# evoldoers/historian

Measured on AMD Instinct MI355X. Metric: forward-DP cells/s, higher is better.
Workload: dtype f64; 1 GPU; batch of independent 2x2000-residue protein leaf-profile pairs, WAG, t=0.2/0.3, full (unbanded) Forward DP; scaled-probability recursion with the reference's truncation: every pairwise sum of the reference's left-nested log_sum_exp drops a term that is at most e^-10 of the other, as the reference's table does (src/logsumexp.h:45); no table, log-probabilities at the store; lpEnd within 1e-9 rel. of; pairs_per_gpu=512, pairs_total=512, parallelism=pairs farmed across 1 rank(s); RCCL broadcast of model constants only

## Files before the change

### historian_amd/csrc/hx_linear.hip

```cpp
#include <hip/hip_runtime.h>
#include <cstdlib>
#include "hx_device.h"
#include "hx_lse.h"
#include "hx_common.h"
#include "hx_policy.h"
#include "hx_kernels.h"

namespace hx {

namespace {

#define HXL_PUBLISH_LAG 16
#define HX_YL_MAX_CLS_LINEAR 64
#define HXL_EMIN (-(1 << 28))
#define HXL_RENORM_MASK 6

struct L5 { double imm, imd, idm, imi, iiw; int e; };

#define HXL_EXP_M10 4.5399929762484854e-05
__device__ __forceinline__ double trunc_sum(double a, double b) {
  const double hi = fmax_plain(a, b), lo = fmin_plain(a, b);
  const int keep = lo > hi * HXL_EXP_M10 ? __double2hiint(lo) : 0;
  return hi + __hiloint2double(keep, __double2loint(lo));
}
template <bool TRUNC> __device__ __forceinline__ double lin_acc(double m, double p, double acc) {
  if (TRUNC) return trunc_sum(acc, m * p);
  return __builtin_fma(m, p, acc);
}

__device__ __forceinline__ L5 l5_zero() { return L5{0., 0., 0., 0., 0., HXL_EMIN}; }

__device__ __forceinline__ int dpp_shr1_keep0(int old, int v) {
  return __builtin_amdgcn_update_dpp(old, v, 0x138, 0xf, 0xf, false);
}
__device__ __forceinline__ double dpp_shr1_keep0(double old, double v) {
  const int lo = __builtin_amdgcn_update_dpp(__double2loint(old), __double2loint(v), 0x138, 0xf, 0xf, false);
  const int hi = __builtin_amdgcn_update_dpp(__double2hiint(old), __double2hiint(v), 0x138, 0xf, 0xf, false);
  return __hiloint2double(hi, lo);
}
__device__ __forceinline__ L5 dpp_shr1_old(const L5& o, const L5& c) {
  return L5{dpp_shr1_keep0(o.imm, c.imm), dpp_shr1_keep0(o.imd, c.imd), dpp_shr1_keep0(o.idm, c.idm),
            dpp_shr1_keep0(o.imi, c.imi), dpp_shr1_keep0(o.iiw, c.iiw), dpp_shr1_keep0(o.e, c.e)};
}

#define HXL_LOG_ENTRIES 1536
typedef double log_entry __attribute__((ext_vector_type(2)));
__device__ __forceinline__ log_entry log_issue(double m, const HX_LDS double* ltab) {
  const double f = __builtin_amdgcn_frexp_mant(m);
  unsigned idx;
  asm("v_bfe_u32 %0, %1, 11, 11" : "=v"(idx) : "v"(__double2hiint(f)));
  return *(const HX_LDS log_entry*)((const HX_LDS char*)ltab + (idx << 4));
}
__device__ __forceinline__ double log_finish(double m, int e, log_entry ce) {
  const double f = __builtin_amdgcn_frexp_mant(m);
  const int k = __builtin_amdgcn_frexp_exp(m);
  const double r = __builtin_fma(f, ce.x, -1.0);
  double p = __builtin_fma(r, 1.0 / 3.0, -0.5);
  p = __builtin_fma(p, r, 1.0);
  const double lf = __builtin_fma(p, r, ce.y);
  return __builtin_fma((double)(e + k), 0.693147180559945309417, lf);
}
__device__ __forceinline__ double log_scaled(double m, int e, const HX_LDS double* ltab) { return log_finish(m, e, log_issue(m, ltab)); }

__device__ __forceinline__ L5 from_logs(double a, double b, double c, double d, double g) {
  const double mx = vmax(vmax(vmax(a, b), vmax(c, d)), g);
  if (!(mx > HX_NEG_INF)) return l5_zero();
  const double n = __builtin_rint(mx * 1.44269504088896340736);
  const double hi = n * 0.693147180369123816490, lo = n * 1.90821492927058770002e-10;
  L5 r;
  r.imm = exp((a - hi) - lo);
  r.imd = exp((b - hi) - lo);
  r.idm = exp((c - hi) - lo);
  r.imi = exp((d - hi) - lo);
  r.iiw = exp((g - hi) - lo);
  r.e = (int)n;
  return r;
}

struct LdsPlan { int elds, ycol, yclass, flags, zero;
                 int a0, b0, a1, stride, total; };

#define HXL_RING 64
#define HXL_STAGE 128

#define HXL_PATIENCE (1 << 22)
template <int W, bool BANDED, int PPW, int DIR, bool MULTI = false, bool TRUNC = false>
__global__ void __launch_bounds__(W * PPW * 64, 4)
k_fill_leaf_linear(const DevJob* __restrict__ jobs, const double* __restrict__ exact_tab, const double* __restrict__ log_tab,
                      const LdsPlan plan, const int n_jobs, const int groups = 1, int* const counters = nullptr) {
  static_assert(!MULTI || (!BANDED && PPW == 1 && W > 1), "several workgroups per pair: unbanded pairs, one pair per workgroup");
  static_assert(!BANDED || W == 1, "banded batches run one wavefront per pair");
  static_assert(PPW == 1 || BANDED, "several pairs per workgroup: banded batches only");
  constexpr int THREADS = W * PPW * 64, PT = W * 64;
  constexpr bool RESCHED = DIR == 0;
  constexpr int RING_ENTRIES = BANDED ? 0 : W * HXL_RING;
  typedef double d2v __attribute__((ext_vector_type(2)));
  extern __shared__ __attribute__((aligned(16))) unsigned char lds[];
  double* ltab = reinterpret_cast<double*>(lds);
  const int pair = PPW == 1 ? 0 : __builtin_amdgcn_readfirstlane((int)(threadIdx.x >> 6));
  const int tid = (int)threadIdx.x - pair * PT;
  const int G = MULTI ? groups : 1;
  const int job = MULTI ? (int)blockIdx.x / G : (int)blockIdx.x * PPW + pair;
  const int grp = MULTI ? (int)blockIdx.x % G : 0;
  const bool live = PPW == 1 || job < n_jobs;
  const DevJob& J = jobs[live ? job : 0];
  unsigned char* blk_a = lds + (pair == 0 ? plan.a0 : plan.a1 + (pair - 1) * plan.stride);
  unsigned char* blk_b = pair == 0 ? lds + plan.b0 : blk_a + (plan.stride - (RING_ENTRIES + HXL_STAGE) * 48);
  double* elds = reinterpret_cast<double*>(blk_a + plan.elds);
  unsigned* ycol = reinterpret_cast<unsigned*>(blk_a + plan.ycol);
  double* yclass = reinterpret_cast<double*>(blk_a + plan.yclass);
  volatile int* prog = reinterpret_cast<volatile int*>(blk_a + plan.flags);
  volatile int* cons = prog + W;
  volatile int* drain = cons + W;
  constexpr bool lds_words = !BANDED;
  for (int k = threadIdx.x; k < 2; k += THREADS) ltab[k] = log_tab[k];
  for (int k = 2048 + threadIdx.x; k < 2 * HXL_LOG_ENTRIES; k += THREADS) ltab[k] = log_tab[k];
  if (tid < 2 * W + 1) prog[tid] = 0;
  if (tid == 0) {
    d2v* z = reinterpret_cast<d2v*>(blk_a + plan.zero);
    z[0] = d2v{0., 0.}; z[1] = d2v{0., 0.}; z[2] = d2v{0., __hiloint2double(0, HXL_EMIN)};
  }
  {
    const int Ky1 = J.y.n_cls + 1, Kx1 = J.x.n_cls + 1;
    for (int jp = tid; jp < (lds_words ? J.n_cols + 130 : 0); jp += PT) {
      const int j = jp < 64 ? 0 : (jp - 64 >= J.n_cols ? J.n_cols - 1 : jp - 64);
      if (BANDED)
        ycol[jp] = (unsigned)J.y.ecls[j] | (J.y.pack[4 * (size_t)j + 3] < 0.0 ? 0x100u : 0u) |
                   ((J.y.flags[j] & F_EDGE) ? 0x200u : 0u) | (J.max_dist >= 0 ? (unsigned)J.y.env[j] << 10 : 0u);
      else if (DIR == 0)
        ycol[jp] = (unsigned)J.y.ecls[j] | (J.y.pack[4 * (size_t)j + 3] < 0.0 ? 0xFFFF0000u : 0u);
      else {
        const int jc = J.n_cols - 1 - j;
        ycol[jp] = (unsigned)J.y.ecls[jc + 1] | (J.y.pack[4 * (size_t)jc + 3] < 0.0 ? 0xFFFF0000u : 0u);
      }
    }
    for (int c = tid; c < Ky1; c += PT) {
      const bool real = c < J.y.n_cls;
      const int rep = real ? J.y.cls_rep[c] : 0;
      yclass[2 * c] = real ? exp(J.y.pack[4 * (size_t)rep + 1]) : 0.;
      yclass[2 * c + 1] = real ? exp(J.y.pack[4 * (size_t)rep + 2]) : 0.;
    }
    for (int e = tid; e < Kx1 * Ky1; e += PT) elds[e] = exp(J.emis_pad[e]);
  }
  __syncthreads();
  const int R = J.n_rows, Cc = J.n_cols;
  const int max_dist = J.max_dist;
  const int lane = threadIdx.x & 63, wave = PPW == 1 ? (RESCHED ? __builtin_amdgcn_readfirstlane((int)(threadIdx.x >> 6)) : (int)(threadIdx.x >> 6)) : 0;
  const int64_t plane = J.plane, ss = J.strip_stride;
  const int blk = J.blk;
  HX_GLOBAL double* __restrict__ M = as_global(DIR ? J.bwd : J.fwd);
  const HX_GLOBAL d4v* xpack = (const HX_GLOBAL d4v*)as_global(J.x.pack);
  double P[5][5];
#pragma unroll
  for (int a = 0; a < 5; ++a)
#pragma unroll
    for (int d = 0; d < 5; ++d) {
      const bool used = d == 0 || (d == 1 && a != 4) || (d == 2 && a != 3) || (d == 3 && (a == 0 || a == 3)) ||
                        (d == 4 && (a == 0 || a == 3 || a == 4));
      if (!used) { P[a][d] = 0.; continue; }
      const double pv = exp(J.T[a][d]);
      double v = __hiloint2double(__builtin_amdgcn_readfirstlane(__double2hiint(pv)), __builtin_amdgcn_readfirstlane(__double2loint(pv)));
      asm volatile("" : "+s"(v));
      P[a][d] = v;
    }
  volatile HX_LDS int* progp = (volatile HX_LDS int*)prog;
  volatile HX_LDS int* consp = (volatile HX_LDS int*)cons;
  volatile HX_LDS int* drainp = (volatile HX_LDS int*)drain;
  const HX_LDS double* lt = (const HX_LDS double*)ltab;
  HX_LDS d2v* ring_mine = (HX_LDS d2v*)blk_b + (size_t)wave * (HXL_RING * 3);
  const int n_strips = live ? (R + 63) / 64 : 0;
  const int prev_wave = (wave + W - 1) % W, next_wave = (wave + 1) % W;
  const int WT = W * G, gw = grp * W + wave;
  HX_GLOBAL int* gdrain = MULTI ? (HX_GLOBAL int*)as_global(counters + 256 * job) : nullptr;
  const int prev_grp = (grp + G - 1) % G;
  bool dead = false;
  const auto wait_drained = [&](const int need) {
    if (!MULTI) {
      while (drainp[0] < need) __builtin_amdgcn_s_sleep(1);
      asm volatile("" ::: "memory");
      return;
    }
    if (dead) return;
    int polls = 0;
    while (__builtin_amdgcn_readfirstlane(__hip_atomic_load(gdrain + prev_grp, __ATOMIC_RELAXED, __HIP_MEMORY_SCOPE_AGENT)) < need) {
      if (++polls > HXL_PATIENCE) {
        dead = true;
        if (lane == 0) __hip_atomic_store(gdrain + 255, 1, __ATOMIC_RELAXED, __HIP_MEMORY_SCOPE_AGENT);
        break;
      }
      __builtin_amdgcn_s_sleep(1);
    }
    asm volatile("" ::: "memory");
  };
  const auto publish_drained = [&](const int value) {
    if (lane != 0) return;
    if (MULTI) __hip_atomic_store(gdrain + grp, value, __ATOMIC_RELAXED, __HIP_MEMORY_SCOPE_AGENT);
    else drainp[0] = value;
  };
  HX_LDS d2v* staging = (HX_LDS d2v*)blk_b + (size_t)RING_ENTRIES * 3;
  const HX_LDS d2v* ring_prev = (const HX_LDS d2v*)blk_b + (size_t)prev_wave * (HXL_RING * 3);

  for (int s = gw; s < n_strips; s += WT) {
    const int row0 = s * 64;
    const int i0 = row0 + lane;
    const bool row_valid = i0 < R;
    double fx, f_imd, f_iiw;
    int x_wait;
    unsigned eoff;
    int env_x = 0;
    bool edge_x = true;
    {
      const int ic = row_valid ? (DIR ? R - 1 - i0 : i0) : 0;
      const d4v p = xpack[ic];
      const d4v q = DIR ? xpack[ic + 1] : p;
      fx = row_valid ? exp(q.x) : 0.;
      f_imd = row_valid ? exp(q.x + q.y) : 0.;
      f_iiw = row_valid ? exp(q.x + q.z) : 0.;
      x_wait = (row_valid && !(p.w < 0.0)) ? 0 : (1 << 29);
      eoff = (unsigned)J.x.ecls[DIR ? ic + 1 : ic] * (unsigned)(J.y.n_cls + 1);
      if (BANDED) {
        env_x = J.max_dist >= 0 ? J.x.env[ic] : 0;
        edge_x = (J.x.flags[ic] & F_EDGE) != 0 || J.max_dist < 0;
      }
    }
    L5 ca = l5_zero(), cb = l5_zero(), ua = l5_zero(), ub = l5_zero();
    const bool has_above = s > 0, has_below = s + 1 < n_strips;
    const bool wrap_in = has_above && wave == 0;
    const bool wrap_out = has_below && wave == W - 1;
    const bool ring_out = has_below && !wrap_out;
    const int above_base = ((s - 1) / WT) * Cc;
    const int my_base = (s / WT) * Cc;
    int64_t store_base = (int64_t)s * ss;
    int store_t0 = 0;
    const int nsteps = (Cc + 64) & ~1;

    auto wait_for = [&](const int cols) {
      const int need = above_base + (cols < Cc ? cols : Cc);
      while (progp[prev_wave] < need) __builtin_amdgcn_s_sleep(1);
      asm volatile("" ::: "memory");
    };
    const HX_LDS d2v* ring_above = !has_above ? (const HX_LDS d2v*)(blk_a + plan.zero) : wrap_in ? (const HX_LDS d2v*)staging : ring_prev;
    const int ring_base = (wrap_in || !has_above) ? 0 : above_base;
    const int ring_mask = !has_above ? 0 : wrap_in ? HXL_STAGE - 1 : HXL_RING - 1;
    auto ring_entry = [&](const int col) -> L5 {
      const HX_LDS d2v* q = ring_above + (size_t)((ring_base + col) & ring_mask) * 3;
      const d2v a = q[0], b = q[1], c = q[2];
      return L5{a.x, a.y, b.x, b.y, c.x, __double2loint(c.y)};
    };
    auto stage_block = [&](const int c0) {
      const int hi = (c0 + 64 < Cc) ? c0 + 64 : Cc;
      const int need = above_base + hi;
      wait_drained(need);
      const int jj = c0 + lane;
      const int64_t sl = jj < Cc ? ((BANDED && DIR == 0) ? stored_slot(J, row0 - 1, jj) : cell_slot_blk(ss, blk, row0 - 1, jj)) : -1;
      if (jj < Cc && sl < 0) {
        HX_LDS d2v* q = staging + (size_t)(jj & (HXL_STAGE - 1)) * 3;
        q[0] = d2v{0., 0.}; q[1] = d2v{0., 0.}; q[2] = d2v{0., __hiloint2double(0, HXL_EMIN)};
      }
      if (sl >= 0) {
        const double a = __hip_atomic_load(M + sl, __ATOMIC_RELAXED, __HIP_MEMORY_SCOPE_AGENT);
        const double b = __hip_atomic_load(M + plane + sl, __ATOMIC_RELAXED, __HIP_MEMORY_SCOPE_AGENT);
        const double c = __hip_atomic_load(M + 2 * plane + sl, __ATOMIC_RELAXED, __HIP_MEMORY_SCOPE_AGENT);
        const double d = __hip_atomic_load(M + 3 * plane + sl, __ATOMIC_RELAXED, __HIP_MEMORY_SCOPE_AGENT);
        const double g = __hip_atomic_load(M + 4 * plane + sl, __ATOMIC_RELAXED, __HIP_MEMORY_SCOPE_AGENT);
        L5 v = from_logs(a, b, c, d, g);
        if (BANDED && max_dist >= 0) {
          const int ia = DIR ? R - row0 : row0 - 1, ja = DIR ? Cc - 1 - jj : jj;
          int dist = J.x.env[ia] - J.y.env[ja];
          dist = dist < 0 ? -dist : dist;
          if (!(((J.x.flags[ia] | J.y.flags[ja]) & F_EDGE) || dist <= max_dist)) v = l5_zero();
        }
        HX_LDS d2v* q = staging + (size_t)(jj & (HXL_STAGE - 1)) * 3;
        q[0] = d2v{v.imm, v.imd};
        q[1] = d2v{v.idm, v.imi};
        q[2] = d2v{v.iiw, __hiloint2double(0, v.e)};
      }
      asm volatile("s_waitcnt lgkmcnt(0)" ::: "memory");
    };
    auto open_sweep = [&](const int t0) {
      if (!has_above) return;
      if (wrap_in) {
        if (t0 > 0 && (t0 & 63) == 0) stage_block(t0 - 64);
        if (t0 < Cc) stage_block(t0 & ~63);
      } else {
        wait_for(8);
      }
      const L5 b0 = ring_entry(t0), bd = ring_entry(t0 > 0 ? t0 - 1 : 0);
      if (lane == 0) {
        ua = b0;
        if (BANDED && t0 > 0) ub = bd;
      }
    };
    unsigned wnext = 0;
    const HX_GLOBAL unsigned* ywords = (const HX_GLOBAL unsigned*)as_global(DIR ? J.yword_bwd : J.yword);
    auto refill_words = [&](const int i0) {
      const unsigned v = ywords[i0 + lane];
      ycol[(i0 + lane) & 255] = v;
      asm volatile("s_waitcnt vmcnt(0) lgkmcnt(0)" ::: "memory");
    };
    auto first_words = [&](const int t0) {
      if (lds_words) { wnext = ycol[t0 + 64 - lane]; return; }
      refill_words(t0 & ~63); refill_words((t0 & ~63) + 64); refill_words((t0 & ~63) + 128);
      wnext = ycol[(t0 + 64 - lane) & 255];
    };
    auto next_word = [&](const int t) -> unsigned {
      const unsigned w = wnext;
      wnext = lds_words ? ycol[t + 65 - lane] : ycol[(t + 65 - lane) & 255];
      return w;
    };
    auto step = [&](const int t, const L5& left, L5& out, L5& u1, L5& u2, const unsigned w) {
      if (!lds_words && (t & 63) == 62) refill_words(t + 2 + 128);
      if ((t & 7) == 7 && has_above && t + 1 < Cc) {
        if (wrap_in) {
          if ((t & 63) == 63) stage_block(t + 1);
        } else {
          if (lane == 0) consp[wave] = above_base + t;
          wait_for(t + 9);
        }
      }
      const unsigned c = BANDED ? (w & 0xFFu) : (w & 0xFFFFu);
      const d2v rc = reinterpret_cast<const d2v*>(yclass)[c];
      const int y_wait = BANDED ? (int)((w & 0x100u) << 21) : (int)((w >> 16) << 13);
      const double em = elds[eoff + c];
      int E;
      if (DIR == 0) {
        double s_imm = u2.imm * P[0][0];
        s_imm = lin_acc<TRUNC>(u2.imd, P[1][0], s_imm);
        s_imm = lin_acc<TRUNC>(u2.idm, P[2][0], s_imm);
        s_imm = lin_acc<TRUNC>(u2.imi, P[3][0], s_imm);
        s_imm = lin_acc<TRUNC>(u2.iiw, P[4][0], s_imm);
        const int e_diag = u2.e;
        __builtin_amdgcn_sched_barrier(0);
        u2 = ring_entry(t + 1);
        __builtin_amdgcn_sched_barrier(0);
        double s_imd = u1.imm * P[0][1];
        double s_iiw = u1.imm * P[0][4];
        double s_idm = left.imm * P[0][2];
        double s_imi = left.imm * P[0][3];
        s_imd = lin_acc<TRUNC>(u1.imd, P[1][1], s_imd);
        s_iiw = lin_acc<TRUNC>(u1.imi, P[3][4], s_iiw);
        s_idm = lin_acc<TRUNC>(left.imd, P[1][2], s_idm);
        s_imi = lin_acc<TRUNC>(left.imi, P[3][3], s_imi);
        s_imd = lin_acc<TRUNC>(u1.idm, P[2][1], s_imd);
        s_iiw = lin_acc<TRUNC>(u1.iiw, P[4][4], s_iiw);
        s_idm = lin_acc<TRUNC>(left.idm, P[2][2], s_idm);
        s_imd = lin_acc<TRUNC>(u1.imi, P[3][1], s_imd);
        s_idm = lin_acc<TRUNC>(left.iiw, P[4][2], s_idm);
        E = left.e > u1.e ? left.e : u1.e;
        E = E > e_diag ? E : e_diag;
        int du = (u1.e - E) - y_wait, dl = (left.e - E) - x_wait, dd = e_diag - E;
        if (BANDED) {
          int dist = env_x - (int)(w >> 10);
          dist = dist < 0 ? -dist : dist;
          const int out_of_env = (edge_x || (w & 0x200u) || dist <= max_dist) ? 0 : (1 << 29);
          du -= out_of_env; dl -= out_of_env; dd -= out_of_env;
        }
        out.imd = __builtin_ldexp(s_imd * f_imd, du);
        out.iiw = __builtin_ldexp(s_iiw * f_iiw, du);
        out.idm = __builtin_ldexp(s_idm * rc.x, dl);
        out.imi = __builtin_ldexp(s_imi * rc.y, dl);
        out.imm = __builtin_ldexp(s_imm * (fx * em), dd);
      } else {
        const int e_diag = u2.e;
        const double tD = u2.imm * (fx * em);
        const double t1x = u1.imd * f_imd, t2x = u1.iiw * f_iiw;
        const double t1y = left.idm * rc.x, t2y = left.imi * rc.y;
        u2 = ring_entry(t + 1);
        E = left.e > u1.e ? left.e : u1.e;
        E = E > e_diag ? E : e_diag;
        int du = (u1.e - E) - y_wait, dl = (left.e - E) - x_wait, dd = e_diag - E;
        if (BANDED) {
          int dist = env_x - (int)(w >> 10);
          dist = dist < 0 ? -dist : dist;
          const int out_of_env = (edge_x || (w & 0x200u) || dist <= max_dist) ? 0 : (1 << 29);
          du -= out_of_env; dl -= out_of_env; dd -= out_of_env;
        }
        const double D = __builtin_ldexp(tD, dd);
        const double d1x = __builtin_ldexp(t1x, du), d2x = __builtin_ldexp(t2x, du);
        const double d1y = __builtin_ldexp(t1y, dl), d2y = __builtin_ldexp(t2y, dl);
        out.imm = lin_acc<TRUNC>(P[0][3], d2y, lin_acc<TRUNC>(P[0][2], d1y, lin_acc<TRUNC>(P[0][4], d2x, lin_acc<TRUNC>(P[0][1], d1x, P[0][0] * D))));
        out.imd = lin_acc<TRUNC>(P[1][2], d1y, lin_acc<TRUNC>(P[1][1], d1x, P[1][0] * D));
        out.idm = lin_acc<TRUNC>(P[2][2], d1y, lin_acc<TRUNC>(P[2][1], d1x, P[2][0] * D));
        out.imi = lin_acc<TRUNC>(P[3][3], d2y, lin_acc<TRUNC>(P[3][4], d2x, lin_acc<TRUNC>(P[3][1], d1x, P[3][0] * D)));
        out.iiw = lin_acc<TRUNC>(P[4][2], d1y, lin_acc<TRUNC>(P[4][4], d2x, P[4][0] * D));
      }
      out.e = E;
      if ((t & HXL_RENORM_MASK) == 0) {
        if (s == 0 && t == 0) {
          if (DIR == 0) {
            if (lane == 0) { out.imm = 1.0; out.e = 0; }
          } else if (lane == 0) {
            const double lpe = J.x.pack[4 * (size_t)R] + J.y.pack[4 * (size_t)Cc];
            out.imm = exp(lpe + J.T[0][5]); out.imd = exp(lpe + J.T[1][5]); out.idm = exp(lpe + J.T[2][5]);
            out.imi = exp(lpe + J.T[3][5]); out.iiw = exp(lpe + J.T[4][5]);
            out.e = 0;
          }
        }
        const double mx = vmax(vmax(vmax(out.imm, out.imd), vmax(out.idm, out.imi)), out.iiw);
        const int k = __builtin_amdgcn_frexp_exp(mx);
        out.imm = __builtin_ldexp(out.imm, -k);
        out.imd = __builtin_ldexp(out.imd, -k);
        out.idm = __builtin_ldexp(out.idm, -k);
        out.imi = __builtin_ldexp(out.imi, -k);
        out.iiw = __builtin_ldexp(out.iiw, -k);
        out.e = mx > 0. ? out.e + k : HXL_EMIN;
      }
      if (ring_out && t >= 63 && t - 63 < Cc) {
        const int col = t - 63;
        if ((col & 7) == 0) {
          const int need = my_base + col + 8 - HXL_RING;
          while (consp[next_wave] < need) __builtin_amdgcn_s_sleep(1);
          asm volatile("" ::: "memory");
        }
        if (lane == 63) {
          HX_LDS d2v* q = ring_mine + (size_t)((my_base + col) & (HXL_RING - 1)) * 3;
          q[0] = d2v{out.imm, out.imd};
          q[1] = d2v{out.idm, out.imi};
          q[2] = d2v{out.iiw, __hiloint2double(0, out.e)};
        }
        if ((col & 7) == 7 || col == Cc - 1) {
          asm volatile("" ::: "memory");
          if (lane == 63) progp[wave] = my_base + col + 1;
        }
      }
      u2 = dpp_shr1_old(u2, out);
    };

    int wlo[2] = {0, 0}, whi[2] = {nsteps, 0};
    if (BANDED) {
      const HX_GLOBAL int32_t* win = as_global(DIR ? J.bwd_windows : J.fwd_windows);
      if (win) {
        for (int w = 0; w < 2; ++w) {
          wlo[w] = win[4 * s + 2 * w] & ~1;
          const int h = (win[4 * s + 2 * w + 1] + 1) & ~1;
          whi[w] = h < nsteps ? h : nsteps;
        }
        if (whi[1] > wlo[1] && wlo[1] <= whi[0]) { whi[0] = whi[1] > whi[0] ? whi[1] : whi[0]; wlo[1] = whi[1] = 0; }
      }
    }
    for (int wi = 0; wi < (BANDED ? 2 : 1); ++wi) {
    if (BANDED && whi[wi] <= wlo[wi]) continue;
    const int wstart = BANDED ? wlo[wi] : 0, wend = BANDED ? whi[wi] : nsteps;
    if (BANDED) { ca = l5_zero(); cb = l5_zero(); ua = l5_zero(); ub = l5_zero(); }
    if (BANDED && DIR == 0 && J.strip_base) { store_base = J.strip_base[2 * s + wi]; store_t0 = wstart; }
    open_sweep(wstart);
    first_words(wstart);
    auto step_pair = [&](const int t) {
      if (RESCHED) {
        step(t, cb, ca, ua, ub, next_word(t));
        const log_entry ea0 = log_issue(ca.imm, lt), ea1 = log_issue(ca.imd, lt), ea2 = log_issue(ca.idm, lt),
                        ea3 = log_issue(ca.imi, lt), ea4 = log_issue(ca.iiw, lt);
        step(t + 1, ca, cb, ub, ua, next_word(t + 1));
        const log_entry eb0 = log_issue(cb.imm, lt), eb1 = log_issue(cb.imd, lt);
        __builtin_amdgcn_sched_barrier(0);
        const double l0 = log_finish(ca.imm, ca.e, ea0), l1 = log_finish(ca.imd, ca.e, ea1);
        const log_entry eb2 = log_issue(cb.idm, lt), eb3 = log_issue(cb.imi, lt);
        __builtin_amdgcn_sched_barrier(0);
        const double l2 = log_finish(ca.idm, ca.e, ea2), l3 = log_finish(ca.imi, ca.e, ea3);
        const log_entry eb4 = log_issue(cb.iiw, lt);
        __builtin_amdgcn_sched_barrier(0);
        const double l4 = log_finish(ca.iiw, ca.e, ea4);
        {
          HX_GLOBAL char* Mu = (HX_GLOBAL char*)(M + (store_base + (int64_t)((t - store_t0) >> 1) * blk));
          unsigned voff = (unsigned)lane << 4;
          asm("" : "+v"(voff));
          const int64_t pb = plane * 8;
          const auto put = [&](const int k, const double l, const double h) {
            const d2v v{l, h};
            if (MULTI) asm volatile("global_store_dwordx4 %0, %1, %2 sc1" ::"v"(voff), "v"(v), "s"(Mu + k * pb) : "memory");
            else __builtin_nontemporal_store(v, (HX_GLOBAL d2v*)(Mu + k * pb + voff));
          };
          const double h0 = log_finish(cb.imm, cb.e, eb0);
          put(0, l0, h0);
          const double h1 = log_finish(cb.imd, cb.e, eb1);
          put(1, l1, h1);
          const double h2 = log_finish(cb.idm, cb.e, eb2);
          put(2, l2, h2);
          const double h3 = log_finish(cb.imi, cb.e, eb3);
          put(3, l3, h3);
          const double h4 = log_finish(cb.iiw, cb.e, eb4);
          put(4, l4, h4);
        }
      } else {
        step(t, cb, ca, ua, ub, next_word(t));
        const double l0 = log_scaled(ca.imm, ca.e, lt), l1 = log_scaled(ca.imd, ca.e, lt),
                     l2 = log_scaled(ca.idm, ca.e, lt), l3 = log_scaled(ca.imi, ca.e, lt),
                     l4 = log_scaled(ca.iiw, ca.e, lt);
        step(t + 1, ca, cb, ub, ua, next_word(t + 1));
        const double h0 = log_scaled(cb.imm, cb.e, lt), h1 = log_scaled(cb.imd, cb.e, lt),
                     h2 = log_scaled(cb.idm, cb.e, lt), h3 = log_scaled(cb.imi, cb.e, lt),
                     h4 = log_scaled(cb.iiw, cb.e, lt);
        HX_GLOBAL d2v* M2 = (HX_GLOBAL d2v*)(M + (store_base + (lane << 1) + (int64_t)((t - store_t0) >> 1) * blk));
        const int64_t plane2 = plane >> 1;
        if (MULTI) {
          const d2v v0{l0, h0}, v1{l1, h1}, v2{l2, h2}, v3{l3, h3}, v4{l4, h4};
          asm volatile("global_store_dwordx4 %0, %1, off sc1" ::"v"(&M2[0]), "v"(v0) : "memory");
          asm volatile("global_store_dwordx4 %0, %1, off sc1" ::"v"(&M2[plane2]), "v"(v1) : "memory");
          asm volatile("global_store_dwordx4 %0, %1, off sc1" ::"v"(&M2[2 * plane2]), "v"(v2) : "memory");
          asm volatile("global_store_dwordx4 %0, %1, off sc1" ::"v"(&M2[3 * plane2]), "v"(v3) : "memory");
          asm volatile("global_store_dwordx4 %0, %1, off sc1" ::"v"(&M2[4 * plane2]), "v"(v4) : "memory");
        } else {
          __builtin_nontemporal_store(d2v{l0, h0}, &M2[0]);
          __builtin_nontemporal_store(d2v{l1, h1}, &M2[plane2]);
          __builtin_nontemporal_store(d2v{l2, h2}, &M2[2 * plane2]);
          __builtin_nontemporal_store(d2v{l3, h3}, &M2[3 * plane2]);
          __builtin_nontemporal_store(d2v{l4, h4}, &M2[4 * plane2]);
        }
      }
      if (wrap_out && !BANDED) {
        const int fin = (t + 2 < nsteps ? t + 2 : nsteps) - 63;
        if (fin >= Cc) {
          asm volatile("s_waitcnt vmcnt(0)" ::: "memory");
          publish_drained(my_base + Cc);
        } else {
          const int done = fin - HXL_PUBLISH_LAG;
          if (done > 0 && ((done >> 6) != ((done - 2) >> 6))) {
            constexpr int PUBLISH_WAIT = 5 * (HXL_PUBLISH_LAG / 2);
            static_assert(PUBLISH_WAIT <= 63 && HXL_PUBLISH_LAG % 2 == 0, "s_waitcnt vmcnt holds 6 bits");
            asm volatile("s_waitcnt vmcnt(%0)" ::"n"(PUBLISH_WAIT) : "memory");
            publish_drained(my_base + done);
          }
        }
      }
    };
    for (int t = wstart; t < wend; t += 2) step_pair(t);
    }
    if (BANDED && wrap_out) {
      asm volatile("s_waitcnt vmcnt(0)" ::: "memory");
      publish_drained(my_base + Cc);
    }
    if (has_above && !wrap_in && lane == 0) consp[wave] = above_base + Cc;
    if (MULTI && s == n_strips - 1) {
      asm volatile("s_waitcnt vmcnt(0)" ::: "memory");
      __builtin_amdgcn_fence(__ATOMIC_ACQUIRE, "agent");
      asm volatile("s_waitcnt vmcnt(0)" ::: "memory");
      const bool gave_up = __hip_atomic_load(gdrain + 255, __ATOMIC_RELAXED, __HIP_MEMORY_SCOPE_AGENT) != 0;
      if (lane == 0) {
        if (DIR == 0) *J.lp_end = gave_up ? __builtin_nan("") : forward_lp_end(J, ExactLse{exact_tab});
        else *J.lp_start = gave_up ? __builtin_nan("") : J.bwd[cell_slot_blk(ss, blk, R - 1, Cc - 1)];
      }
    }
  }
  if (MULTI) return;
  asm volatile("s_waitcnt vmcnt(0)" ::: "memory");
  __syncthreads();
  if (live && wave == 0 && lane == 0) {
    if (DIR == 0) *J.lp_end = forward_lp_end(J, ExactLse{exact_tab});
    else *J.lp_start = J.bwd[cell_slot_blk(ss, blk, R - 1, Cc - 1)];
  }
}

}

int log_table_doubles() { return 2 * HXL_LOG_ENTRIES; }
void build_log_table(double* out) {
  for (int k = 0; k < 2 * HXL_LOG_ENTRIES; ++k) out[k] = 0.;
  out[1] = -HUGE_VAL;
  for (int k = 0; k < 512; ++k) {
    const double centre = 0.5 * (1.0 + (k + 0.5) / 512.0);
    const double c = 1.0 / centre;
    out[2 * (1024 + k)] = c;
    out[2 * (1024 + k) + 1] = -log(c);
  }
}

static LdsPlan plan_lds(int W, int PPW, bool banded, int yl_cols, int yl_emis, int yl_cls) {
  LdsPlan p;
  const int table = 16 * HXL_LOG_ENTRIES, hole = 16 * 1024;
  int a = 0;
  p.elds = a; a += (8 * yl_emis + 15) & ~15;
  p.ycol = a; a += banded ? 4 * 256 : (4 * (yl_cols + 132) + 15) & ~15;
  p.yclass = a; a += 16 * yl_cls;
  p.flags = a; a += (4 * (2 * W + 1) + 15) & ~15;
  p.zero = a; a += 48;
  const int b = ((banded ? 0 : W * HXL_RING) + HXL_STAGE) * 48;
  int end = table;
  if (16 + a + b <= hole) { p.a0 = 16; p.b0 = 16 + a; }
  else if (16 + a <= hole) { p.a0 = 16; p.b0 = end; end += b; }
  else { p.a0 = end; p.b0 = end + a; end += a + b; }
  p.a1 = end;
  p.stride = a + b;
  end += (PPW - 1) * p.stride;
  p.total = (end + 15) & ~15;
  return p;
}

int launch_forward_leaf_linear(const DevJob* d_jobs, int n_jobs, int max_rows, bool banded, Tab8 tab8, Tab16 tab16,
                               int yl_cols, int yl_emis, int yl_cls, int multi, int* counters, bool trunc, hipStream_t st) {
  const double* tab = tab8.p;
  const double* log_tab = tab16.p;
  if (yl_cls > HX_YL_MAX_CLS_LINEAR + 1) return launch_fail("%d emission classes exceed the scaled-probability kernel's column words", yl_cls);
  if (multi > 1 && !banded) {
    const LdsPlan p = plan_lds(4, 1, false, yl_cols, yl_emis, yl_cls);
    if (p.total > HX_LDS_LIMIT) return launch_fail("k_fill_leaf_linear<multi> needs %d bytes of LDS (limit %d)", p.total, HX_LDS_LIMIT);
    if (trunc)
      hipLaunchKernelGGL((k_fill_leaf_linear<4, false, 1, 0, true, true>), dim3(n_jobs * multi), dim3(4 * 64), p.total, st, d_jobs, tab, log_tab, p, n_jobs,
                         multi, counters);
    else
      hipLaunchKernelGGL((k_fill_leaf_linear<4, false, 1, 0, true>), dim3(n_jobs * multi), dim3(4 * 64), p.total, st, d_jobs, tab, log_tab, p, n_jobs,
                         multi, counters);
    return 0;
  }
#define HXL_LAUNCH(W_, B_, PPW_) do { const LdsPlan p = plan_lds(W_, PPW_, B_, yl_cols, yl_emis, yl_cls); \
    if (p.total > HX_LDS_LIMIT) return launch_fail("k_fill_leaf_linear<%d> needs %d bytes of LDS (limit %d)", W_, p.total, HX_LDS_LIMIT); \
    if (trunc) hipLaunchKernelGGL((k_fill_leaf_linear<W_, B_, PPW_, 0, false, true>), dim3((n_jobs + PPW_ - 1) / PPW_), dim3(W_ * PPW_ * 64), p.total, st, \
                       d_jobs, tab, log_tab, p, n_jobs); \
    else hipLaunchKernelGGL((k_fill_leaf_linear<W_, B_, PPW_, 0>), dim3((n_jobs + PPW_ - 1) / PPW_), dim3(W_ * PPW_ * 64), p.total, st, \
                       d_jobs, tab, log_tab, p, n_jobs); } while (0)
  if (banded) {
    const char* v = getenv("HX_LINEAR_PPW");
    const int forced = v ? atoi(v) : 0;
    if (forced > 1 || (forced == 0 && n_jobs > 1024)) {
      if (plan_lds(1, 6, true, yl_cols, yl_emis, yl_cls).total <= 76 * 1024) HXL_LAUNCH(1, true, 6);
      else if (plan_lds(1, 5, true, yl_cols, yl_emis, yl_cls).total <= 76 * 1024) HXL_LAUNCH(1, true, 5);
      else HXL_LAUNCH(1, true, 4);
    } else HXL_LAUNCH(1, true, 1);
    return 0;
  }
  const char* v = getenv("HX_LINEAR_WAVES");
  const int forced = v ? atoi(v) : 0;
  if (forced == 1) HXL_LAUNCH(1, false, 1);
  else if (forced == 2) HXL_LAUNCH(2, false, 1);
  else if (forced == 4) HXL_LAUNCH(4, false, 1);
  else if (forced == 8) HXL_LAUNCH(8, false, 1);
  else if (forced == 16) HXL_LAUNCH(16, false, 1);
  else if (max_rows <= 64) HXL_LAUNCH(1, false, 1);
  else if (max_rows <= 128) HXL_LAUNCH(2, false, 1);
  else if (max_rows <= 256) HXL_LAUNCH(4, false, 1);
  else if (max_rows <= 512 || n_jobs > 256) HXL_LAUNCH(8, false, 1);
  else HXL_LAUNCH(16, false, 1);
#undef HXL_LAUNCH
  return 0;
}

int launch_backward_leaf_linear(const DevJob* d_jobs, int n_jobs, int max_rows, bool banded, Tab8 tab8, Tab16 tab16,
                                int yl_cols, int yl_emis, int yl_cls, int multi, int* counters, bool trunc, hipStream_t st) {
  const double* tab = tab8.p;
  const double* log_tab = tab16.p;
  if (yl_cls > HX_YL_MAX_CLS_LINEAR + 1) return launch_fail("%d emission classes exceed the scaled-probability kernel's column words", yl_cls);
  if (multi > 1 && !banded) {
    const LdsPlan p = plan_lds(4, 1, false, yl_cols, yl_emis, yl_cls);
    if (p.total > HX_LDS_LIMIT) return launch_fail("k_fill_leaf_linear<multi> needs %d bytes of LDS (limit %d)", p.total, HX_LDS_LIMIT);
    if (trunc)
      hipLaunchKernelGGL((k_fill_leaf_linear<4, false, 1, 1, true, true>), dim3(n_jobs * multi), dim3(4 * 64), p.total, st, d_jobs, tab, log_tab, p, n_jobs,
                         multi, counters);
    else
      hipLaunchKernelGGL((k_fill_leaf_linear<4, false, 1, 1, true>), dim3(n_jobs * multi), dim3(4 * 64), p.total, st, d_jobs, tab, log_tab, p, n_jobs,
                         multi, counters);
    return 0;
  }
#define HXL_LAUNCH(W_, B_, PPW_) do { const LdsPlan p = plan_lds(W_, PPW_, B_, yl_cols, yl_emis, yl_cls); \
    if (p.total > HX_LDS_LIMIT) return launch_fail("k_fill_leaf_linear<%d, bwd> needs %d bytes of LDS (limit %d)", W_, p.total, HX_LDS_LIMIT); \
    if (trunc) hipLaunchKernelGGL((k_fill_leaf_linear<W_, B_, PPW_, 1, false, true>), dim3((n_jobs + PPW_ - 1) / PPW_), dim3(W_ * PPW_ * 64), p.total, st, \
                       d_jobs, tab, log_tab, p, n_jobs); \
    else hipLaunchKernelGGL((k_fill_leaf_linear<W_, B_, PPW_, 1>), dim3((n_jobs + PPW_ - 1) / PPW_), dim3(W_ * PPW_ * 64), p.total, st, \
                       d_jobs, tab, log_tab, p, n_jobs); } while (0)
  if (banded) {
    const char* v = getenv("HX_LINEAR_PPW");
    const int forced = v ? atoi(v) : 0;
    if (forced > 1 || (forced == 0 && n_jobs > 1024)) {
      if (plan_lds(1, 6, true, yl_cols, yl_emis, yl_cls).total <= 76 * 1024) HXL_LAUNCH(1, true, 6);
      else if (plan_lds(1, 5, true, yl_cols, yl_emis, yl_cls).total <= 76 * 1024) HXL_LAUNCH(1, true, 5);
      else HXL_LAUNCH(1, true, 4);
    } else HXL_LAUNCH(1, true, 1);
    return 0;
  }
  const char* v = getenv("HX_LINEAR_WAVES");
  const int forced = v ? atoi(v) : 0;
  if (forced == 1) HXL_LAUNCH(1, false, 1);
  else if (forced == 2) HXL_LAUNCH(2, false, 1);
  else if (forced == 8) HXL_LAUNCH(8, false, 1);
  else if (max_rows <= 64) HXL_LAUNCH(1, false, 1);
  else if (max_rows <= 128) HXL_LAUNCH(2, false, 1);
  else if (max_rows <= 256) HXL_LAUNCH(4, false, 1);
  else if (max_rows <= 512 || n_jobs > 256) HXL_LAUNCH(8, false, 1);
  else HXL_LAUNCH(16, false, 1);
#undef HXL_LAUNCH
  return 0;
}

}
```

Baseline: 115.4 billion cells/s.

## Hand over pre-multiplied upper-row sums in forward linear fill

For the forward direction, each cell now precomputes the three transition-weighted sums (match, delete, wait) that the row below needs. It passes those downstream through the DPP shift and the LDS ring instead of the five raw states, which cuts ring traffic and the per-step dependent multiply-adds. The forward wave index is also remapped for W>4, and s_nop padding is added after the MULTI stores. The hand-over duplicates the transition arithmetic in the producer, and truncation order changes slightly, which could shift numerics.

```diff
diff --git a/historian_amd/csrc/hx_linear.hip b/historian_amd/csrc/hx_linear.hip
--- a/historian_amd/csrc/hx_linear.hip
+++ b/historian_amd/csrc/hx_linear.hip
@@ -30,6 +30,11 @@
 
 __device__ __forceinline__ L5 l5_zero() { return L5{0., 0., 0., 0., 0., HXL_EMIN}; }
 
+struct S3 { double imm, imd, iiw; int e; };
+__device__ __forceinline__ S3 s3_zero() { return S3{0., 0., 0., HXL_EMIN}; }
+template <int DIR> struct HandOver { typedef S3 type; static __device__ __forceinline__ S3 zero() { return s3_zero(); } };
+template <> struct HandOver<1> { typedef L5 type; static __device__ __forceinline__ L5 zero() { return l5_zero(); } };
+
 __device__ __forceinline__ int dpp_shr1_keep0(int old, int v) {
   return __builtin_amdgcn_update_dpp(old, v, 0x138, 0xf, 0xf, false);
 }
@@ -41,6 +46,9 @@
 __device__ __forceinline__ L5 dpp_shr1_old(const L5& o, const L5& c) {
   return L5{dpp_shr1_keep0(o.imm, c.imm), dpp_shr1_keep0(o.imd, c.imd), dpp_shr1_keep0(o.idm, c.idm),
             dpp_shr1_keep0(o.imi, c.imi), dpp_shr1_keep0(o.iiw, c.iiw), dpp_shr1_keep0(o.e, c.e)};
+}
+__device__ __forceinline__ S3 dpp_shr1_old(const S3& o, const S3& c) {
+  return S3{dpp_shr1_keep0(o.imm, c.imm), dpp_shr1_keep0(o.imd, c.imd), dpp_shr1_keep0(o.iiw, c.iiw), dpp_shr1_keep0(o.e, c.e)};
 }
 
 #define HXL_LOG_ENTRIES 1536
@@ -95,6 +103,7 @@
   constexpr bool RESCHED = DIR == 0;
   constexpr int RING_ENTRIES = BANDED ? 0 : W * HXL_RING;
   typedef double d2v __attribute__((ext_vector_type(2)));
+  typedef typename HandOver<DIR>::type UP;
   extern __shared__ __attribute__((aligned(16))) unsigned char lds[];
   double* ltab = reinterpret_cast<double*>(lds);
   const int pair = PPW == 1 ? 0 : __builtin_amdgcn_readfirstlane((int)(threadIdx.x >> 6));
@@ -118,7 +127,7 @@
   if (tid < 2 * W + 1) prog[tid] = 0;
   if (tid == 0) {
     d2v* z = reinterpret_cast<d2v*>(blk_a + plan.zero);
-    z[0] = d2v{0., 0.}; z[1] = d2v{0., 0.}; z[2] = d2v{0., __hiloint2double(0, HXL_EMIN)};
+    z[0] = d2v{0., 0.}; z[1] = d2v{0., DIR == 0 ? __hiloint2double(0, HXL_EMIN) : 0.}; z[2] = d2v{0., __hiloint2double(0, HXL_EMIN)};
   }
   {
     const int Ky1 = J.y.n_cls + 1, Kx1 = J.x.n_cls + 1;
@@ -145,7 +154,8 @@
   __syncthreads();
   const int R = J.n_rows, Cc = J.n_cols;
   const int max_dist = J.max_dist;
-  const int lane = threadIdx.x & 63, wave = PPW == 1 ? (RESCHED ? __builtin_amdgcn_readfirstlane((int)(threadIdx.x >> 6)) : (int)(threadIdx.x >> 6)) : 0;
+  const int lane = threadIdx.x & 63, hw_wave = PPW == 1 ? (RESCHED ? __builtin_amdgcn_readfirstlane((int)(threadIdx.x >> 6)) : (int)(threadIdx.x >> 6)) : 0;
+  const int wave = (DIR == 0 && W > 4) ? (hw_wave ^ ((hw_wave & 4) ? 3 : 0)) : hw_wave;
   const int64_t plane = J.plane, ss = J.strip_stride;
   const int blk = J.blk;
   HX_GLOBAL double* __restrict__ M = as_global(DIR ? J.bwd : J.fwd);
@@ -223,7 +233,8 @@
         edge_x = (J.x.flags[ic] & F_EDGE) != 0 || J.max_dist < 0;
       }
     }
-    L5 ca = l5_zero(), cb = l5_zero(), ua = l5_zero(), ub = l5_zero();
+    L5 ca = l5_zero(), cb = l5_zero();
+    UP ua = HandOver<DIR>::zero(), ub = HandOver<DIR>::zero();
     const bool has_above = s > 0, has_below = s + 1 < n_strips;
     const bool wrap_in = has_above && wave == 0;
     const bool wrap_out = has_below && wave == W - 1;
@@ -242,10 +253,39 @@
     const HX_LDS d2v* ring_above = !has_above ? (const HX_LDS d2v*)(blk_a + plan.zero) : wrap_in ? (const HX_LDS d2v*)staging : ring_prev;
     const int ring_base = (wrap_in || !has_above) ? 0 : above_base;
     const int ring_mask = !has_above ? 0 : wrap_in ? HXL_STAGE - 1 : HXL_RING - 1;
-    auto ring_entry = [&](const int col) -> L5 {
+    auto ring_entry = [&](const int col) -> UP {
       const HX_LDS d2v* q = ring_above + (size_t)((ring_base + col) & ring_mask) * 3;
-      const d2v a = q[0], b = q[1], c = q[2];
-      return L5{a.x, a.y, b.x, b.y, c.x, __double2loint(c.y)};
+      if constexpr (DIR == 0) {
+        const d2v a = q[0], b = q[1];
+        return S3{a.x, a.y, b.x, __double2loint(b.y)};
+      } else {
+        const d2v a = q[0], b = q[1], c = q[2];
+        return L5{a.x, a.y, b.x, b.y, c.x, __double2loint(c.y)};
+      }
+    };
+    auto hand_over = [&](const L5& c) -> S3 {
+      double s_imm = c.imm * P[0][0], s_imd = c.imm * P[0][1], s_iiw = c.imm * P[0][4];
+      s_imm = lin_acc<TRUNC>(c.imd, P[1][0], s_imm);
+      s_imd = lin_acc<TRUNC>(c.imd, P[1][1], s_imd);
+      s_iiw = lin_acc<TRUNC>(c.imi, P[3][4], s_iiw);
+      s_imm = lin_acc<TRUNC>(c.idm, P[2][0], s_imm);
+      s_imd = lin_acc<TRUNC>(c.idm, P[2][1], s_imd);
+      s_iiw = lin_acc<TRUNC>(c.iiw, P[4][4], s_iiw);
+      s_imm = lin_acc<TRUNC>(c.imi, P[3][0], s_imm);
+      s_imd = lin_acc<TRUNC>(c.imi, P[3][1], s_imd);
+      s_imm = lin_acc<TRUNC>(c.iiw, P[4][0], s_imm);
+      return S3{s_imm, s_imd, s_iiw, c.e};
+    };
+    auto put_entry = [&](HX_LDS d2v* q, const L5& c) {
+      if constexpr (DIR == 0) {
+        const S3 h = hand_over(c);
+        q[0] = d2v{h.imm, h.imd};
+        q[1] = d2v{h.iiw, __hiloint2double(0, h.e)};
+      } else {
+        q[0] = d2v{c.imm, c.imd};
+        q[1] = d2v{c.idm, c.imi};
+        q[2] = d2v{c.iiw, __hiloint2double(0, c.e)};
+      }
     };
     auto stage_block = [&](const int c0) {
       const int hi = (c0 + 64 < Cc) ? c0 + 64 : Cc;
@@ -255,7 +295,7 @@
       const int64_t sl = jj < Cc ? ((BANDED && DIR == 0) ? stored_slot(J, row0 - 1, jj) : cell_slot_blk(ss, blk, row0 - 1, jj)) : -1;
       if (jj < Cc && sl < 0) {
         HX_LDS d2v* q = staging + (size_t)(jj & (HXL_STAGE - 1)) * 3;
-        q[0] = d2v{0., 0.}; q[1] = d2v{0., 0.}; q[2] = d2v{0., __hiloint2double(0, HXL_EMIN)};
+        q[0] = d2v{0., 0.}; q[1] = d2v{0., DIR == 0 ? __hiloint2double(0, HXL_EMIN) : 0.}; q[2] = d2v{0., __hiloint2double(0, HXL_EMIN)};
       }
       if (sl >= 0) {
         const double a = __hip_atomic_load(M + sl, __ATOMIC_RELAXED, __HIP_MEMORY_SCOPE_AGENT);
@@ -270,10 +310,7 @@
           dist = dist < 0 ? -dist : dist;
           if (!(((J.x.flags[ia] | J.y.flags[ja]) & F_EDGE) || dist <= max_dist)) v = l5_zero();
         }
-        HX_LDS d2v* q = staging + (size_t)(jj & (HXL_STAGE - 1)) * 3;
-        q[0] = d2v{v.imm, v.imd};
-        q[1] = d2v{v.idm, v.imi};
-        q[2] = d2v{v.iiw, __hiloint2double(0, v.e)};
+        put_entry(staging + (size_t)(jj & (HXL_STAGE - 1)) * 3, v);
       }
       asm volatile("s_waitcnt lgkmcnt(0)" ::: "memory");
     };
@@ -285,7 +322,7 @@
       } else {
         wait_for(8);
       }
-      const L5 b0 = ring_entry(t0), bd = ring_entry(t0 > 0 ? t0 - 1 : 0);
+      const UP b0 = ring_entry(t0), bd = ring_entry(t0 > 0 ? t0 - 1 : 0);
       if (lane == 0) {
         ua = b0;
         if (BANDED && t0 > 0) ub = bd;
@@ -308,7 +345,7 @@
       wnext = lds_words ? ycol[t + 65 - lane] : ycol[(t + 65 - lane) & 255];
       return w;
     };
-    auto step = [&](const int t, const L5& left, L5& out, L5& u1, L5& u2, const unsigned w) {
+    auto step = [&](const int t, const L5& left, L5& out, UP& u1, UP& u2, const unsigned w) {
       if (!lds_words && (t & 63) == 62) refill_words(t + 2 + 128);
       if ((t & 7) == 7 && has_above && t + 1 < Cc) {
         if (wrap_in) {
@@ -323,28 +360,17 @@
       const int y_wait = BANDED ? (int)((w & 0x100u) << 21) : (int)((w >> 16) << 13);
       const double em = elds[eoff + c];
       int E;
-      if (DIR == 0) {
-        double s_imm = u2.imm * P[0][0];
-        s_imm = lin_acc<TRUNC>(u2.imd, P[1][0], s_imm);
-        s_imm = lin_acc<TRUNC>(u2.idm, P[2][0], s_imm);
-        s_imm = lin_acc<TRUNC>(u2.imi, P[3][0], s_imm);
-        s_imm = lin_acc<TRUNC>(u2.iiw, P[4][0], s_imm);
+      if constexpr (DIR == 0) {
+        const double s_imm = u2.imm, s_imd = u1.imd, s_iiw = u1.iiw;
         const int e_diag = u2.e;
         __builtin_amdgcn_sched_barrier(0);
         u2 = ring_entry(t + 1);
         __builtin_amdgcn_sched_barrier(0);
-        double s_imd = u1.imm * P[0][1];
-        double s_iiw = u1.imm * P[0][4];
         double s_idm = left.imm * P[0][2];
         double s_imi = left.imm * P[0][3];
-        s_imd = lin_acc<TRUNC>(u1.imd, P[1][1], s_imd);
-        s_iiw = lin_acc<TRUNC>(u1.imi, P[3][4], s_iiw);
         s_idm = lin_acc<TRUNC>(left.imd, P[1][2], s_idm);
         s_imi = lin_acc<TRUNC>(left.imi, P[3][3], s_imi);
-        s_imd = lin_acc<TRUNC>(u1.idm, P[2][1], s_imd);
-        s_iiw = lin_acc<TRUNC>(u1.iiw, P[4][4], s_iiw);
         s_idm = lin_acc<TRUNC>(left.idm, P[2][2], s_idm);
-        s_imd = lin_acc<TRUNC>(u1.imi, P[3][1], s_imd);
         s_idm = lin_acc<TRUNC>(left.iiw, P[4][2], s_idm);
         E = left.e > u1.e ? left.e : u1.e;
         E = E > e_diag ? E : e_diag;
@@ -388,6 +414,7 @@
       if ((t & HXL_RENORM_MASK) == 0) {
         if (s == 0 && t == 0) {
           if (DIR == 0) {
+            asm volatile("" : "+v"(out.imm), "+v"(out.e));
             if (lane == 0) { out.imm = 1.0; out.e = 0; }
           } else if (lane == 0) {
             const double lpe = J.x.pack[4 * (size_t)R] + J.y.pack[4 * (size_t)Cc];
@@ -405,6 +432,8 @@
         out.iiw = __builtin_ldexp(out.iiw, -k);
         out.e = mx > 0. ? out.e + k : HXL_EMIN;
       }
+      UP mine;
+      if constexpr (DIR == 0) mine = hand_over(out); else mine = out;
       if (ring_out && t >= 63 && t - 63 < Cc) {
         const int col = t - 63;
         if ((col & 7) == 0) {
@@ -414,16 +443,21 @@
         }
         if (lane == 63) {
           HX_LDS d2v* q = ring_mine + (size_t)((my_base + col) & (HXL_RING - 1)) * 3;
-          q[0] = d2v{out.imm, out.imd};
-          q[1] = d2v{out.idm, out.imi};
-          q[2] = d2v{out.iiw, __hiloint2double(0, out.e)};
+          if constexpr (DIR == 0) {
+            q[0] = d2v{mine.imm, mine.imd};
+            q[1] = d2v{mine.iiw, __hiloint2double(0, mine.e)};
+          } else {
+            q[0] = d2v{out.imm, out.imd};
+            q[1] = d2v{out.idm, out.imi};
+            q[2] = d2v{out.iiw, __hiloint2double(0, out.e)};
+          }
         }
         if ((col & 7) == 7 || col == Cc - 1) {
           asm volatile("" ::: "memory");
           if (lane == 63) progp[wave] = my_base + col + 1;
         }
       }
-      u2 = dpp_shr1_old(u2, out);
+      u2 = dpp_shr1_old(u2, mine);
     };
 
     int wlo[2] = {0, 0}, whi[2] = {nsteps, 0};
@@ -441,7 +475,7 @@
     for (int wi = 0; wi < (BANDED ? 2 : 1); ++wi) {
     if (BANDED && whi[wi] <= wlo[wi]) continue;
     const int wstart = BANDED ? wlo[wi] : 0, wend = BANDED ? whi[wi] : nsteps;
-    if (BANDED) { ca = l5_zero(); cb = l5_zero(); ua = l5_zero(); ub = l5_zero(); }
+    if (BANDED) { ca = l5_zero(); cb = l5_zero(); ua = HandOver<DIR>::zero(); ub = HandOver<DIR>::zero(); }
     if (BANDED && DIR == 0 && J.strip_base) { store_base = J.strip_base[2 * s + wi]; store_t0 = wstart; }
     open_sweep(wstart);
     first_words(wstart);
@@ -467,7 +501,7 @@
           const int64_t pb = plane * 8;
           const auto put = [&](const int k, const double l, const double h) {
             const d2v v{l, h};
-            if (MULTI) asm volatile("global_store_dwordx4 %0, %1, %2 sc1" ::"v"(voff), "v"(v), "s"(Mu + k * pb) : "memory");
+            if (MULTI) asm volatile("global_store_dwordx4 %0, %1, %2 sc1\n\ts_nop 1" ::"v"(voff), "v"(v), "s"(Mu + k * pb) : "memory");
             else __builtin_nontemporal_store(v, (HX_GLOBAL d2v*)(Mu + k * pb + voff));
           };
           const double h0 = log_finish(cb.imm, cb.e, eb0);
@@ -494,11 +528,11 @@
         const int64_t plane2 = plane >> 1;
         if (MULTI) {
           const d2v v0{l0, h0}, v1{l1, h1}, v2{l2, h2}, v3{l3, h3}, v4{l4, h4};
-          asm volatile("global_store_dwordx4 %0, %1, off sc1" ::"v"(&M2[0]), "v"(v0) : "memory");
-          asm volatile("global_store_dwordx4 %0, %1, off sc1" ::"v"(&M2[plane2]), "v"(v1) : "memory");
-          asm volatile("global_store_dwordx4 %0, %1, off sc1" ::"v"(&M2[2 * plane2]), "v"(v2) : "memory");
-          asm volatile("global_store_dwordx4 %0, %1, off sc1" ::"v"(&M2[3 * plane2]), "v"(v3) : "memory");
-          asm volatile("global_store_dwordx4 %0, %1, off sc1" ::"v"(&M2[4 * plane2]), "v"(v4) : "memory");
+          asm volatile("global_store_dwordx4 %0, %1, off sc1\n\ts_nop 1" ::"v"(&M2[0]), "v"(v0) : "memory");
+          asm volatile("global_store_dwordx4 %0, %1, off sc1\n\ts_nop 1" ::"v"(&M2[plane2]), "v"(v1) : "memory");
+          asm volatile("global_store_dwordx4 %0, %1, off sc1\n\ts_nop 1" ::"v"(&M2[2 * plane2]), "v"(v2) : "memory");
+          asm volatile("global_store_dwordx4 %0, %1, off sc1\n\ts_nop 1" ::"v"(&M2[3 * plane2]), "v"(v3) : "memory");
+          asm volatile("global_store_dwordx4 %0, %1, off sc1\n\ts_nop 1" ::"v"(&M2[4 * plane2]), "v"(v4) : "memory");
         } else {
           __builtin_nontemporal_store(d2v{l0, h0}, &M2[0]);
           __builtin_nontemporal_store(d2v{l1, h1}, &M2[plane2]);
```

Measured after the change: 116.5 billion cells/s (median of 6 runs). About the same (+0.9%).
